# fanzhongyi/diffusion

Hardware: AMD Instinct MI355X
Metric: U-Net training images/sec @256 (SD-2-base U-Net, precomputed latents 4x32x32) (higher is better)
Workload: dtype bf16; 1 GPU; SD-2-base U-Net train step, latents 4x32x32, text 77x1024, batch 256/GPU (global 256), microbatch 256, AdamW, dp1; global_batch=256, microbatch=256, parallelism=dp1, params=865910724

## Files before the change

### diffusion_amd/_lib.py

```python
from __future__ import annotations

import ctypes as C
import os

_HERE = os.path.dirname(os.path.abspath(__file__))
LIB_PATH = os.path.join(_HERE, os.environ.get('DA_LIB_ALT') or 'libdiffusion_amd.so')

_vp, _l, _i, _f, _fp, _ll = C.c_void_p, C.c_long, C.c_int, C.c_float, C.c_void_p, C.c_void_p

SIGNATURES = {
    'da_gemm_nt': [_vp, _l, _vp, _vp, _l, _fp, _vp, _l, _vp, _l, _i, _i, _i, _i, _i, _i, _i, _i, _i, _i, _i, _f, _fp, _l,
                   _vp],
    'da_set_option': [C.c_char_p, _i],
    'da_gemm_nt_variant_for': [_i, _i, _i, _i, _l],
    'da_gemm_nt_geglu': [_vp, _l, _vp, _vp, _l, _vp, _l, _fp, _i, _i, _i, _vp],
    'da_gemm_nt_geglu_bwd': [_vp, _l, _vp, _vp, _l, _vp, _l, _i, _i, _i, _vp],
    'da_gemm_tn_wgrad': [_vp, _l, _vp, _l, _fp, _fp, _fp, _i, _i, _i, _i, _i, _i, _i, _i, _i, _fp, _l, _vp],
    'da_gemm_tn_variant_for': [_i, _i, _i, _i, _i, _i, _i, _i, _i],
    'da_attn_fwd': [_vp, _l, _vp, _l, _vp, _l, _vp, _l, _fp, _i, _i, _i, _i, _f, _vp],
    'da_attn_fwd_causal': [_vp, _l, _vp, _l, _vp, _l, _vp, _l, _fp, _i, _i, _i, _f, _vp],
    'da_attn_bwd': [_vp, _l, _vp, _l, _vp, _l, _vp, _l, _vp, _l, _fp, _fp, _vp, _l, _vp, _l, _vp, _l, _i, _i, _i, _i,
                    _f, _vp],
    'da_norm_scratch_floats': [_i, _i, _i],
    'da_groupnorm_fwd': [_vp, _l, _vp, _l, _fp, _fp, _fp, _fp, _fp, _i, _i, _i, _i, _f, _i, _vp],
    'da_groupnorm_bwd': [_vp, _l, _vp, _l, _vp, _l, _vp, _l, _fp, _fp, _fp, _fp, _fp, _fp, _fp, _i, _i, _i, _i, _i,
                         _vp],
    'da_groupnorm_plan_for': [_i, _i, _i, _i, _l, _l, _i, C.POINTER(_i)],
    'da_layernorm_fwd': [_vp, _l, _vp, _l, _fp, _fp, _fp, _i, _i, _f, _vp],
    'da_layernorm_bwd': [_vp, _l, _vp, _l, _vp, _l, _vp, _l, _fp, _fp, _fp, _fp, _fp, _i, _i, _vp],
    'da_colsum_accum': [_vp, _l, _fp, _fp, _i, _i, _vp],
    'da_image_colsum': [_vp, _l, _vp, _l, _fp, _fp, _i, _i, _i, _vp],
    'da_geglu_fwd': [_vp, _l, _vp, _l, _i, _i, _vp],
# ... 60 lines not shown
```

### diffusion_amd/csrc/gemm_tn.hip

```cpp
#include "common.hpp"
#include "diffusion_amd.h"

namespace {

struct GemmTNParams {
  const bf16* dY;
  const bf16* X;
  float* dW;
  long lddy, ldx;
  int M, N, Kt, Cin;
  int Hin, Win, Hout, Wout, ksize, mode;
  FastDiv div_hw, div_w;
  int tiles_n, tiles_k, splits, m_per_split;
  float* slab;
  int overwrite;
};

constexpr int TN_BM = 32;
constexpr int TN_LD = 288;
constexpr int TN_TILE = TN_BM * TN_LD;
constexpr int TN_STAGE = 2 * TN_TILE;
constexpr int TN_SMEM = 2 * TN_STAGE;

__global__ __launch_bounds__(256, 2) void gemm_tn_kernel(GemmTNParams p) {
// ... 153 lines not shown
      for (int u = 0; u < 8; ++u) acc[u] += *reinterpret_cast<const f32x4*>(src + (long)(sp + u) * 128 * 128);
    }
    for (int u = 0; sp < p.splits; ++sp, ++u) acc[u & 7] += *reinterpret_cast<const f32x4*>(src + (long)sp * 128 * 128);
    f32x4* dst = reinterpret_cast<f32x4*>(p.dW + (long)n * p.Kt + kc);
    const f32x4 sum = ((acc[0] + acc[1]) + (acc[2] + acc[3])) + ((acc[4] + acc[5]) + (acc[6] + acc[7]));
    *dst = p.overwrite ? sum : *dst + sum;
  }
}

}

int da_gemm_tn_v2_dispatch(int variant, const void* dY, long lddy, const void* X, long ldx, float* dW, float* dbias,
                           int M, int N, int Cin, int Hin, int Win, int Hout, int Wout, int ksize, int mode, float* ws,
                           long ws_floats, hipStream_t stream);
int da_gemm_tn_v2_fast_period(int M, int N, int Hin, int Win, int Hout, int Wout, int mode);
int g_tn_variant = 0;
int g_grad_overwrite = 0;

static bool tn_takes_v2(int M, int N, int Kt) {
  const bool big = (N >= 160) && (Kt >= 256) && (M >= 1024 || (M >= 256 && (long)N * Kt >= (8L << 20)));
  return g_tn_variant == 2 || g_tn_variant == 3 || (g_tn_variant == 0 && big);
}

extern "C" int da_gemm_tn_variant_for(int M, int N, int Cin, int Hin, int Win, int Hout, int Wout, int ksize, int mode) {
  if (!tn_takes_v2(M, N, ksize * ksize * Cin)) return 1;
  return da_gemm_tn_v2_fast_period(M, N, Hin, Win, Hout, Wout, mode) ? 3 : 2;
}

extern "C" int da_gemm_tn_wgrad(const void* dY, long lddy, const void* X, long ldx, float* dW, float* dbias,
                                float* scratch, int M, int N, int Cin, int Hin, int Win, int Hout, int Wout, int ksize,
// ... 39 lines not shown
  p.slab = nullptr;
  p.overwrite = g_grad_overwrite;
  if (splits > 1 && split_ws && (long)tiles * splits * 128 * 128 <= split_ws_floats && (p.Kt & 3) == 0) p.slab = split_ws;
  if (p.overwrite && splits > 1 && !p.slab)
    if (hipMemsetAsync(dW, 0, (size_t)N * p.Kt * sizeof(float), stream) != hipSuccess) return DA_ERR_LAUNCH;
  hipLaunchKernelGGL(gemm_tn_kernel, dim3(tiles * splits), dim3(256), 0, stream, p);
  DA_CHECK_LAUNCH();
  if (p.slab) {
    long blocks = ((long)p.N * (p.Kt >> 2) + 255) / 256;
    if (blocks > 2048) blocks = 2048;
    hipLaunchKernelGGL(tn1_slab_reduce_kernel, dim3((int)blocks), dim3(256), 0, stream, p);
    DA_CHECK_LAUNCH();
  }
  return DA_OK;
}
```

### diffusion_amd/csrc/gemm_tn_v2.hip

```cpp
#include "common.hpp"
#include "diffusion_amd.h"

int da_usable_cus(int cus);
extern int g_grad_overwrite;
int g_tn_ring = 0;


namespace {

struct GemmTN2Params {
  const bf16* dY;
  const bf16* X;
  float* dW;
  float* dbias;
  long lddy, ldx;
  int M, N, Kt, Cin;
  int Hin, Win, Hout, Wout, ksize, mode;
  FastDiv div_hw, div_w, div_cin;
  int tiles_n, tiles_k, splits, m_per_split;
  float* slab;
  float* bslab;
  int overwrite;
  int period;
  int ups64;
// ... 4 lines not shown
constexpr int T2_MS = 64;
constexpr int T2_BN = 320;
constexpr int T2_SA = T2_BN * 2;
constexpr int T2_A_BYTES = T2_MS * T2_SA;
constexpr int T2_AJ = T2_A_BYTES / 1024 / 8;

DEVINL int swA(int row) { return 2 * ((row >> 1) & 3); }
template <int BK>
DEVINL int swB(int row) { return (BK * 2) % 256 == 0 ? 2 * (row & 7) : 2 * ((row >> 1) & 3); }

DEVINL void glds16_tn(const void* gsrc, char* lds_dst) {
  __builtin_amdgcn_global_load_lds((const __attribute__((address_space(1))) void*)gsrc,
                                   (__attribute__((address_space(3))) void*)lds_dst, 16, 0, 0);
}

template <int T2_BK, bool FAST, bool CT, int RING = 0>
__global__ __launch_bounds__(512, 2) void gemm_tn2_kernel(GemmTN2Params p) {
  constexpr int T2_SB = T2_BK * 2;
  constexpr int T2_B_BYTES = T2_MS * T2_SB;
  constexpr int T2_STAGE = T2_A_BYTES + T2_B_BYTES;
  constexpr int T2_BJ = T2_B_BYTES / 1024 / 8;
  constexpr int C16B = T2_SB / 16;
  constexpr int JT = T2_BK / 32;
  extern __shared__ __attribute__((aligned(16))) char smem[];
  const int tid = threadIdx.x;
  const int lane = tid & 63;
  const int wave = __builtin_amdgcn_readfirstlane(tid >> 6);
  const int wa = wave >> 1, wb = wave & 1;

  int bid = blockIdx.x;
  {
    const int nblk = p.tiles_n * p.tiles_k * p.splits;
    const int q = nblk >> 3, r = nblk & 7;
    const int xcd = bid & 7, idx = bid >> 3;
    bid = (xcd < r ? xcd * (q + 1) : r * (q + 1) + (xcd - r) * q) + idx;
  }
  const int tk = bid % p.tiles_k;
  bid /= p.tiles_k;
  const int split = bid % p.splits;
  const int tn = bid / p.splits;
  const int n0 = tn * T2_BN, k0 = tk * T2_BK;
  const int m_begin = split * p.m_per_split;
  const int m_end = min(p.M, m_begin + p.m_per_split);
  const int nsteps = (m_end - m_begin + T2_MS - 1) / T2_MS;
  if (nsteps <= 0) return;
  const int HWo = p.Hout * p.Wout;
  const int pad = (p.ksize == 3) ? 1 : 0;
  const int gmul = (p.mode == 1) ? 2 : 1, gshift = (p.mode == 3) ? 1 : 0;
  const int hlim = (p.mode == 3) ? p.Hout : p.Hin, wlim = (p.mode == 3) ? p.Wout : p.Win;
  const char* zero = reinterpret_cast<const char*>(g_zero_page_tn);

  int mcur_f = m_begin;
  unsigned fa_off[T2_AJ], fx_off[T2_BJ], fx_off1[T2_BJ], fx_m0[T2_BJ], fx_m1[T2_BJ];
  const int src_step = (int)((long)T2_MS * p.Hin * p.Win / HWo);
  const long x_margin = (long)pad * (p.Win + 1);
// ... 221 lines not shown
#pragma unroll
      for (int i = 0; i < 5; ++i)
#pragma unroll
        for (int jj = 0; jj < JT / 2; ++jj)
          acc[i][jh * (JT / 2) + jj] =
              CT ? __builtin_amdgcn_mfma_f32_16x16x32_bf16(bfr[jj], a[i], acc[i][jh * (JT / 2) + jj], 0, 0, 0)
                 : __builtin_amdgcn_mfma_f32_16x16x32_bf16(a[i], bfr[jj], acc[i][jh * (JT / 2) + jj], 0, 0, 0);
    }
  };

  auto compute_half = [&](int stage, int ms) {
    const unsigned Ab = smem_off + stage * T2_STAGE;
    compute_half_at(Ab, Ab + T2_A_BYTES, ms);
  };

  if constexpr (RING > 0) {
    static_assert(!RING || (FAST && T2_BK == 192), "ring form: linear layers on the FAST path, 4 pieces per wave and half");
    constexpr int HALF_A = 32 * T2_SA, HALF = HALF_A + 32 * T2_SB;
    const int nh = (m_end - m_begin) >> 5;
    const bool is_a = wave < 5;
    unsigned off[4];
#pragma unroll
    for (int j = 0; j < 4; ++j) {
      if (is_a) {
        const int ci = (wave * 4 + j) * 64 + lane;
        const int row = ci / 40, pc = ci - row * 40;
        const int n = min(n0 + (pc ^ swA(row)) * 8, p.N - 8);
        off[j] = (unsigned)(row * (int)p.lddy + n);
      } else {
        const int ci = ((wave - 5) * 4 + j) * 64 + lane;
// ... 16 lines not shown
    };
#pragma unroll
    for (int h = 0; h < RING - 1; ++h) issue_half();
    int slot = 0;
    for (int h = 0; h < nh; ++h) {
      asm volatile("s_waitcnt vmcnt(%0)\n\ts_barrier" ::"n"(4 * (RING - 2)) : "memory");
      issue_half();
      const unsigned Ab = smem_off + slot * HALF;
      compute_half_at(Ab, Ab + HALF_A, 0);
      slot = slot + 1 == RING ? 0 : slot + 1;
    }
    asm volatile("s_waitcnt vmcnt(0)" ::: "memory");
  } else if constexpr (FAST) {
    issue_fast(0, true);
    __syncthreads();
    for (int t = 0; t < nsteps; ++t) {
      issue_fast((t + 1) & 1, t + 1 < nsteps);
      compute_half(t & 1, 0);
      compute_half(t & 1, 1);
      __syncthreads();
    }
  } else {
    issue(0);
    __syncthreads();
    for (int t = 0; t < nsteps; ++t) {
      compute_half(t & 1, 0);
      if (t + 1 < nsteps) issue((t + 1) & 1);
      compute_half(t & 1, 1);
      __syncthreads();
    }
  }

  if constexpr (CT) {
#pragma unroll
    for (int i = 0; i < 5; ++i)
#pragma unroll
      for (int j = 0; j < JT; ++j) {
        const int nl = wa * 80 + i * 16 + (lane & 15), kl = wb * (16 * JT) + j * 16 + (lane >> 4) * 4;
        const int n = n0 + nl, kc = k0 + kl;
        if (p.slab && p.splits > 1) {
          *reinterpret_cast<f32x4*>(p.slab + (((long)(tn * p.tiles_k + tk) * p.splits + split) * T2_BN + nl) * T2_BK + kl) = acc[i][j];
        } else if (n < p.N && kc < p.Kt) {
          float* dst = p.dW + (long)n * p.Kt + kc;
          if (p.splits == 1) {
            if (p.overwrite) *reinterpret_cast<f32x4*>(dst) = acc[i][j];
            else *reinterpret_cast<f32x4*>(dst) += acc[i][j];
          } else {
#pragma unroll
            for (int e = 0; e < 4; ++e) unsafeAtomicAdd(dst + e, acc[i][j][e]);
          }
        }
      }
    if (do_bias && lane < 16) {
#pragma unroll
      for (int i = 0; i < 5; ++i) {
        const int nl = wa * 80 + i * 16 + lane, n = n0 + nl;
        if (p.slab && p.splits > 1) p.bslab[((long)tn * p.splits + split) * T2_BN + nl] = accb[i][0];
        else if (n < p.N) {
          if (p.splits == 1) p.dbias[n] = p.overwrite ? accb[i][0] : p.dbias[n] + accb[i][0];
          else unsafeAtomicAdd(p.dbias + n, accb[i][0]);
        }
      }
    }
    return;
  }
#pragma unroll
  for (int i = 0; i < 5; ++i)
#pragma unroll
    for (int j = 0; j < JT; ++j) {
      const int kc = k0 + wb * (16 * JT) + j * 16 + (lane & 15);
#pragma unroll
      for (int e = 0; e < 4; ++e) {
        const int n = n0 + wa * 80 + i * 16 + (lane >> 4) * 4 + e;
        if (p.slab && p.splits > 1) {
          const int nl = wa * 80 + i * 16 + (lane >> 4) * 4 + e, kl = wb * (16 * JT) + j * 16 + (lane & 15);
          p.slab[(((long)(tn * p.tiles_k + tk) * p.splits + split) * T2_BN + nl) * T2_BK + kl] = acc[i][j][e];
        } else if (n < p.N && kc < p.Kt) {
          float* dst = p.dW + (long)n * p.Kt + kc;
          if (p.splits == 1) *dst = p.overwrite ? acc[i][j][e] : *dst + acc[i][j][e];
          else unsafeAtomicAdd(dst, acc[i][j][e]);
        }
      }
    }
  if (do_bias && (lane & 15) == 0) {
#pragma unroll
    for (int i = 0; i < 5; ++i)
#pragma unroll
      for (int e = 0; e < 4; ++e) {
        const int nl = wa * 80 + i * 16 + (lane >> 4) * 4 + e, n = n0 + nl;
        if (p.slab && p.splits > 1) p.bslab[((long)tn * p.splits + split) * T2_BN + nl] = accb[i][e];
        else if (n < p.N) {
          if (p.splits == 1) p.dbias[n] = p.overwrite ? accb[i][e] : p.dbias[n] + accb[i][e];
          else unsafeAtomicAdd(p.dbias + n, accb[i][e]);
        }
      }
  }
}

template <int BK>
__global__ __launch_bounds__(256) void tn_slab_reduce_kernel(GemmTN2Params p, int main_blocks) {
  if ((int)blockIdx.x >= main_blocks) {
    const int grp = threadIdx.x >> 4, l = threadIdx.x & 15;
    const int n = ((int)blockIdx.x - main_blocks) * 16 + grp;
    if (n < p.N) {
      const int tn = n / T2_BN;
      const float* src = p.bslab + ((long)tn * p.splits) * T2_BN + (n - tn * T2_BN);
      float a0 = 0.f, a1 = 0.f;
      int sp = l;
      for (; sp + 16 < p.splits; sp += 32) {
        a0 += src[(long)sp * T2_BN];
// ... 17 lines not shown
    f32x4 acc[8];
#pragma unroll
    for (int u = 0; u < 8; ++u) acc[u] = f32x4{0.f, 0.f, 0.f, 0.f};
    int sp = 0;
    for (; sp + 7 < p.splits; sp += 8) {
#pragma unroll
      for (int u = 0; u < 8; ++u) acc[u] += *reinterpret_cast<const f32x4*>(src + (long)(sp + u) * T2_BN * BK);
    }
    for (int u = 0; sp < p.splits; ++sp, ++u) acc[u & 7] += *reinterpret_cast<const f32x4*>(src + (long)sp * T2_BN * BK);
    f32x4* dst = reinterpret_cast<f32x4*>(p.dW + (long)n * p.Kt + kc);
    const f32x4 sum = ((acc[0] + acc[1]) + (acc[2] + acc[3])) + ((acc[4] + acc[5]) + (acc[6] + acc[7]));
    *dst = p.overwrite ? sum : *dst + sum;
  }
}

template <int BK, bool FAST>
int launch_tn2(GemmTN2Params p, float* ws, long ws_floats, hipStream_t stream) {
  constexpr int SMEM = 2 * (T2_A_BYTES + T2_MS * BK * 2);
  p.tiles_n = (p.N + T2_BN - 1) / T2_BN;
  p.tiles_k = (p.Kt + BK - 1) / BK;
  const int tiles = p.tiles_n * p.tiles_k;
  const int ncu = da_usable_cus(256);
  int best = 1;
  if (tiles < (ncu * 29) / 32) {
    int kcap = p.M / 6000;
    const int one_round = (ncu + tiles - 1) / tiles;
    if (kcap < one_round) kcap = one_round;
    const int max_splits = p.M / 512 > 0 ? p.M / 512 : 1;
    if (kcap > max_splits) kcap = max_splits;
    double best_eff = -1.0;
    bool found = false;
    for (int k = 1; k <= kcap; ++k) {
      const long blocks = (long)tiles * k;
      const double eff = (double)blocks / (double)(((blocks + ncu - 1) / ncu) * ncu);
      if (eff >= 0.9 && blocks >= ncu - 6) {
        best = k;
        found = true;
        break;
      }
      if (eff >= best_eff - 1e-9) {
        best_eff = eff;
        best = k;
      }
    }
    (void)found;
  }
  int mps = (p.M + best - 1) / best;
  mps = ((mps + T2_MS - 1) / T2_MS) * T2_MS;
  p.splits = (p.M + mps - 1) / mps;
  p.m_per_split = mps;
  static unsigned long long attr_done = 0, attr_done_ct = 0;
  if (da_ensure_dyn_smem((const void*)gemm_tn2_kernel<BK, FAST, false>, SMEM, &attr_done) != DA_OK) return DA_ERR_LAUNCH;
  if (da_ensure_dyn_smem((const void*)gemm_tn2_kernel<BK, FAST, true>, SMEM, &attr_done_ct) != DA_OK) return DA_ERR_LAUNCH;
  p.slab = p.bslab = nullptr;
  {
    const long tile_floats = (long)tiles * p.splits * T2_BN * BK;
    const long bias_floats = p.dbias ? (long)p.tiles_n * p.splits * T2_BN : 0;
    if (p.splits > 1 && ws && tile_floats + bias_floats <= ws_floats && (p.Kt & 3) == 0) {
      p.slab = ws;
      p.bslab = ws + tile_floats;
    }
// ... 59 lines not shown
  p.dY = (const bf16*)dY; p.X = (const bf16*)X; p.dW = dW; p.dbias = dbias;
  p.lddy = lddy; p.ldx = ldx;
  p.M = M; p.N = N; p.Cin = Cin; p.Kt = ksize * ksize * Cin;
  p.Hin = Hin; p.Win = Win; p.Hout = Hout; p.Wout = Wout; p.ksize = ksize; p.mode = mode;
  p.div_hw = make_fastdiv((unsigned)(Hout * Wout));
  p.div_w = make_fastdiv((unsigned)Wout);
  p.div_cin = make_fastdiv((unsigned)Cin);
  p.tiles_n = p.tiles_k = p.splits = p.m_per_split = 0;
  p.slab = p.bslab = nullptr;
  p.overwrite = 0;
  (void)variant;
  p.period = da_gemm_tn_v2_fast_period(M, N, Hin, Win, Hout, Wout, mode);
  p.ups64 = (p.period && mode == 3 && Wout == T2_MS) ? 1 : 0;
  return p.period ? launch_tn2<192, true>(p, ws, ws_floats, stream) : launch_tn2<192, false>(p, ws, ws_floats, stream);
}
```

### diffusion_amd/models/unet.py

```python
from __future__ import annotations

import math
import os
from dataclasses import dataclass
from typing import Dict, List, Optional, Tuple

import torch
import torch.nn as nn

from .. import ops
from ..ops import BF16, F32, Geom


@dataclass
class UNetConfig:
    in_channels: int = 4
    out_channels: int = 4
    block_out_channels: Tuple[int, ...] = (320, 640, 1280, 1280)
    attention_head_dim: Tuple[int, ...] = (5, 10, 20, 20)
    cross_attention_dim: int = 1024
    layers_per_block: int = 2
    norm_num_groups: int = 32
    norm_eps: float = 1e-5
    sample_size: int = 64
# ... 229 lines not shown
        fp = self.fp
        self.master = torch.zeros(fp.total, device=dev, dtype=F32)
        self.grad = torch.zeros(fp.total, device=dev, dtype=F32)
        self.exp_avg = torch.zeros(fp.total, device=dev, dtype=F32)
        self.exp_avg_sq = torch.zeros(fp.total, device=dev, dtype=F32)
        self.shadow = torch.zeros(fp.total, device=dev, dtype=BF16)
        self.shadow_t = torch.zeros(max(fp.total_t, 8), device=dev, dtype=BF16)
        self._bind_views()
        self._scratch = None
        self._scratch_key = None
        self.opt_step = 0
        self._grad_fresh = False
        self._grad_ready_cb = None
        import os
        self.wgrad_stream = torch.cuda.Stream() if os.environ.get('DA_WGRAD_STREAM', '0') == '1' else None
        self._tape = None
        if init:
            self.reset_parameters(seed)

    def _bind_views(self):
        fp = self.fp
        self._mats: Dict[str, Mat] = {}
        self._vecs: Dict[str, Vec] = {}
        for name, st in fp.storages.items():
            sl = slice(st.off, st.off + st.numel)
            if st.ntc is not None:
                N, T, C = st.ntc
                m = Mat()
                m.N, m.T, m.C = N, T, C
                m.w = self.shadow[sl].view(N, T * C)
# ... 147 lines not shown
            return
        main = torch.cuda.current_stream()
        ev = torch.cuda.Event()
        ev.record(main)
        ws.wait_event(ev)
        dy.record_stream(ws)
        x.record_stream(ws)
        with torch.cuda.stream(ws):
            old = ops.SPLITK_WS
            ops.SPLITK_WS = self._wgrad_ws
            try:
                ops.gemm_tn_wgrad(dy, x, gw, g, dbias=dbias, scratch=self._wgrad_scratch if scratch is not None else None)
            finally:
                ops.SPLITK_WS = old

    def _lin_fwd(self, x, key, out=None, bias=True, residual=None):
        m = self.M(key + '.weight')
        M = x.shape[0]
        y = out if out is not None else self._bf(M, m.N)
        ops.gemm_nt(x, m.w, y, Geom.linear(M), bias=self.V(key + '.bias').p if bias else None, residual=residual)
        return y

    def _lin_bwd(self, x, dy, key, bias=True, need_dx=True, dx_out=None):
        m = self.M(key + '.weight')
        M = x.shape[0]
        if _DGRAD_FIRST and need_dx:
            dx = dx_out if dx_out is not None else self._bf(M, m.C)
            ops.gemm_nt(dy, m.wt, dx, Geom.linear(M))
            self._wgrad(dy, x, m.gw, Geom.linear(M), dbias=self.V(key + '.bias').g if bias else None, scratch=self._scratch)
            return dx
        self._wgrad(dy, x, m.gw, Geom.linear(M), dbias=self.V(key + '.bias').g if bias else None,
                          scratch=self._scratch)
        if not need_dx:
            return None
        dx = dx_out if dx_out is not None else self._bf(M, m.C)
        ops.gemm_nt(dy, m.wt, dx, Geom.linear(M))
        return dx

    def _resnet_fwd(self, p, x, B, H, W, out=None):
        cfg = self.cfg
# ... 92 lines not shown
            ops.geglu_fwd(f, gg)
        h3 = self._lin_fwd(gg, tb + '.ff.net.2', residual=h2)
        y = self._lin_fwd(h3, p + '.proj_out', out=out, residual=x)
        saved = (p, x, gst, g, h0, ln1, n1, qkv, o1, l1, h1, ln2, n2, q2, kv2, o2, l2, h2, ln3, n3, f, gg, h3, B, H, W,
                 heads)
        return y, saved

    def _transformer_bwd(self, saved, dout):
        (p, x, gst, g, h0, ln1, n1, qkv, o1, l1, h1, ln2, n2, q2, kv2, o2, l2, h2, ln3, n3, f, gg, h3, B, H, W,
         heads) = saved
        HW = H * W
        M = B * HW
        C = x.shape[1]
        tb = p + '.transformer_blocks.0'
        nk = self._ctx.shape[0] // B
        dh3 = self._lin_bwd(h3, dout, p + '.proj_out')
        df = self._bf(M, 8 * C)
        if ops.geglu_bwd_fusable(4 * C, C):
            self._lin_bwd(gg, dh3, tb + '.ff.net.2', need_dx=False)
            ops.gemm_nt_geglu_bwd(dh3, self.M(tb + '.ff.net.2.weight').wt, f, df)
        else:
            dgg = self._lin_bwd(gg, dh3, tb + '.ff.net.2')
            ops.geglu_bwd(f, dgg, df)
            del dgg
        dn3 = self._lin_bwd(n3, df, tb + '.ff.net.0.proj')
        del df
        dh2 = self._ln_bwd(h2, dn3, dh3, tb + '.norm3', ln3)
        do2 = self._lin_bwd(o2, dh2, tb + '.attn2.to_out.0')
        dq2 = self._bf(M, C)
        dkv2 = self._bf(B * nk, 2 * C)
        ops.attn_bwd(q2, kv2[:, :C], kv2[:, C:], o2, do2, l2, self._delta, dq2, dkv2[:, :C], dkv2[:, C:], B, heads, HW,
                     nk, 0.125)
        self._wgrad(dkv2, self._ctx, self.M(tb + '.attn2.kv.weight').gw, Geom.linear(B * nk))
        dn2 = self._lin_bwd(n2, dq2, tb + '.attn2.to_q', bias=False)
        dh1 = self._ln_bwd(h1, dn2, dh2, tb + '.norm2', ln2)
        do1 = self._lin_bwd(o1, dh1, tb + '.attn1.to_out.0')
        dqkv = self._bf(M, 3 * C)
        ops.attn_bwd(qkv[:, :C], qkv[:, C:2 * C], qkv[:, 2 * C:], o1, do1, l1, self._delta, dqkv[:, :C],
                     dqkv[:, C:2 * C], dqkv[:, 2 * C:], B, heads, HW, HW, 0.125)
        mq = self.M(tb + '.attn1.qkv.weight')
        self._wgrad(dqkv, n1, mq.gw, Geom.linear(M))
        dn1 = self._bf(M, C)
        ops.gemm_nt(dqkv, mq.wt, dn1, Geom.linear(M))
        dh0 = self._ln_bwd(h0, dn1, dh1, tb + '.norm1', ln1)
        dg = self._lin_bwd(g, dh0, p + '.proj_in')
        return self._gn_bwd(x, dg, dout, p + '.norm', gst, B, HW, 0)

    def forward_features(self, xt8: torch.Tensor, t: torch.Tensor, ctx: torch.Tensor, B: int, S: int):
        cfg = self.cfg
        boc = cfg.block_out_channels
        n = len(boc)
        self._ensure_scratch(B, S)
        self._ctx = ctx
        tape: List[Tuple[str, tuple]] = []
        te0 = self._bf(B, boc[0])
        if t.dtype == F32:
            ops.timestep_embed_f32(t, te0)
        else:
            ops.timestep_embed(t, te0)
        te1 = self._lin_fwd(te0, 'time_embedding.linear_1')
# ... 216 lines not shown
```

### diffusion_amd/ops.py

```python
from __future__ import annotations

import ctypes
import os
from typing import Optional, Tuple

import torch

from . import _lib

BF16 = torch.bfloat16
F32 = torch.float32


def _stream() -> int:
    return torch.cuda.current_stream().cuda_stream


SPLITK_WS = None


PROFILE = None


class _Timed:
# ... 181 lines not shown
    if M != g.B * g.Hout * g.Wout or X.shape[0] != g.B * g.Hin * g.Win:
        raise ValueError('wgrad: row counts do not match the geometry')
    if dW.dtype != F32 or not dW.is_contiguous() or dW.numel() != N * g.ksize * g.ksize * Cin:
        raise ValueError(f'dW must be contiguous fp32 with {N * g.ksize * g.ksize * Cin} elements')
    mode = g.mode
    if mode == 2:
        raise ValueError('wgrad has no mode 2')
    with _Timed('gemm_tn', 2.0 * M * N * g.ksize * g.ksize * Cin, (M, N, g.ksize * g.ksize * Cin, g.ksize, g.mode)):
        db = _vec(dbias, N, 'dbias') if dbias is not None else 0
        sc = _f32buf(scratch, 256 * N * 2, 'scratch') if dbias is not None else 0
        _lib.call('da_gemm_tn_wgrad', dy_ptr, lddy, x_ptr, ldx, dW.data_ptr(), db, sc, M, N, Cin, g.Hin, g.Win,
                  g.Hout, g.Wout, g.ksize, mode, SPLITK_WS.data_ptr() if SPLITK_WS is not None else 0,
                  SPLITK_WS.numel() if SPLITK_WS is not None else 0, _stream())


def attn_fwd(Q, K, V, O, L2, B, H, Nq, Nk, scale):
    q, ldq = _mat(Q, BF16, 'Q')
    k, ldk = _mat(K, BF16, 'K')
    v, ldv = _mat(V, BF16, 'V')
    o, ldo = _mat(O, BF16, 'O')
    for t, n in ((Q, Nq), (O, Nq), (K, Nk), (V, Nk)):
        if tuple(t.shape) != (B * n, H * 64):
            raise ValueError(f'attention operand shape {tuple(t.shape)} != {(B * n, H * 64)}')
    with _Timed('attn_fwd', 4.0 * B * H * Nq * Nk * 64, (B, H, Nq, Nk, 0)):
        _lib.call('da_attn_fwd', q, ldq, k, ldk, v, ldv, o, ldo, _f32buf(L2, B * H * Nq, 'L2'), B, H, Nq, Nk,
                  float(scale), _stream())


def attn_fwd_causal(Q, K, V, O, L2, B, H, N, scale):
    q, ldq = _mat(Q, BF16, 'Q')
# ... 283 lines not shown
```

### include/diffusion_amd.h

```cpp
#ifndef DIFFUSION_AMD_H
#define DIFFUSION_AMD_H

#ifdef __cplusplus
extern "C" {
#endif

typedef struct ihipStream_t* da_stream_t;

int da_gemm_nt(const void* A, long lda, const void* W, void* C, long ldc, const float* bias, const void* rowbias,
               long ldrb, const void* R, long ldr, int M, int N, int K, int Cin, int Hin, int Win, int Hout, int Wout,
               int ksize, int mode, int out_fp32, float alpha, float* splitk_ws, long splitk_ws_floats,
               da_stream_t stream);

int da_gemm_nt_geglu(const void* A, long lda, const void* W, void* F, long ldf, void* G, long ldg, const float* bias,
                     int M, int inner, int K, da_stream_t stream);

int da_gemm_nt_geglu_bwd(const void* dY, long lddy, const void* Wt, const void* F, long ldf, void* dF, long lddf, int M,
                         int inner, int K, da_stream_t stream);

int da_set_option(const char* key, int value);
int da_gemm_nt_variant_for(int M, int N, int K, int Cin, long splitk_ws_floats);

int da_gemm_tn_wgrad(const void* dY, long lddy, const void* X, long ldx, float* dW, float* dbias, float* scratch, int M,
                     int N, int Cin, int Hin, int Win, int Hout, int Wout, int ksize, int mode, float* split_ws,
                     long split_ws_floats, da_stream_t stream);

int da_gemm_tn_variant_for(int M, int N, int Cin, int Hin, int Win, int Hout, int Wout, int ksize, int mode);

int da_attn_fwd(const void* Q, long ldq, const void* K, long ldk, const void* V, long ldv, void* O, long ldo,
                float* L2, int B, int H, int Nq, int Nk, float scale, da_stream_t stream);
int da_attn_fwd_causal(const void* Q, long ldq, const void* K, long ldk, const void* V, long ldv, void* O, long ldo,
                       float* L2, int B, int H, int N, float scale, da_stream_t stream);
int da_attn_bwd(const void* Q, long ldq, const void* K, long ldk, const void* V, long ldv, const void* O, long ldo,
                const void* dO, long lddo, const float* L2, float* Delta, void* dQ, long lddq, void* dK, long lddk,
                void* dV, long lddv, int B, int H, int Nq, int Nk, float scale, da_stream_t stream);

long da_norm_scratch_floats(int B, int HW, int C);

int da_groupnorm_fwd(const void* X, long ldx, void* Y, long ldy, const float* gamma, const float* beta,
                     float* mean_rstd, float* scale_shift, float* scratch, int B, int HW, int C, int G, float eps,
// ... 64 lines not shown
```

Baseline: 1538 images/sec.

## Batch transformer-block weight-gradient GEMMs into one grouped split-K launch

Defers the weight-gradient GEMMs of each transformer block's linear layers (proj_in/out, attention projections, FF) and runs them together in one grouped TN kernel, followed by a single split-K reduction kernel. Tiles from all problems share one grid, so the GPU fills better than with many small separate launches, and per-launch overhead drops. The tile kernel also gains a periodic accumulator flush into the slab or output during the main loop. The costs are extra workspace traffic, keeping activations alive longer, and more complex dispatch with a fallback to per-problem launches.

```diff
diff --git a/diffusion_amd/_lib.py b/diffusion_amd/_lib.py
--- a/diffusion_amd/_lib.py
+++ b/diffusion_amd/_lib.py
@@ -16,6 +16,7 @@
     'da_gemm_nt_geglu': [_vp, _l, _vp, _vp, _l, _vp, _l, _fp, _i, _i, _i, _vp],
     'da_gemm_nt_geglu_bwd': [_vp, _l, _vp, _vp, _l, _vp, _l, _i, _i, _i, _vp],
     'da_gemm_tn_wgrad': [_vp, _l, _vp, _l, _fp, _fp, _fp, _i, _i, _i, _i, _i, _i, _i, _i, _i, _fp, _l, _vp],
+    'da_gemm_tn_wgrad_grouped': [_vp, _i, _i, _fp, _l, _vp],
     'da_gemm_tn_variant_for': [_i, _i, _i, _i, _i, _i, _i, _i, _i],
     'da_attn_fwd': [_vp, _l, _vp, _l, _vp, _l, _vp, _l, _fp, _i, _i, _i, _i, _f, _vp],
     'da_attn_fwd_causal': [_vp, _l, _vp, _l, _vp, _l, _vp, _l, _fp, _i, _i, _i, _f, _vp],
diff --git a/diffusion_amd/csrc/gemm_tn.hip b/diffusion_amd/csrc/gemm_tn.hip
--- a/diffusion_amd/csrc/gemm_tn.hip
+++ b/diffusion_amd/csrc/gemm_tn.hip
@@ -191,6 +191,7 @@
                            int M, int N, int Cin, int Hin, int Win, int Hout, int Wout, int ksize, int mode, float* ws,
                            long ws_floats, hipStream_t stream);
 int da_gemm_tn_v2_fast_period(int M, int N, int Hin, int Win, int Hout, int Wout, int mode);
+int da_gemm_tn_v2_group(const DaWgradProblem* pr, int n, int M, float* ws, long ws_floats, hipStream_t stream);
 int g_tn_variant = 0;
 int g_grad_overwrite = 0;
 
@@ -260,3 +261,37 @@
   }
   return DA_OK;
 }
+
+extern "C" int da_gemm_tn_wgrad_grouped(const DaWgradProblem* pr, int n, int M, float* ws, long ws_floats, hipStream_t stream) {
+  DA_CLEAR_ERR();
+  if (!pr || n <= 0 || M <= 0 || M >= (1 << 24)) return DA_ERR_SHAPE;
+  if (!ws) ws_floats = 0;
+  bool group = g_tn_variant == 0;
+  for (int i = 0; i < n; ++i) {
+    const DaWgradProblem& q = pr[i];
+    if (!q.dY || !q.X || !q.dW || q.N <= 0 || q.Cin <= 0) return DA_ERR_SHAPE;
+    if ((q.N & 7) || (q.Cin & 7) || (q.lddy & 7) || (q.ldx & 7)) return DA_ERR_SHAPE;
+    group = group && tn_takes_v2(M, q.N, q.Cin) && da_gemm_tn_v2_fast_period(M, q.N, 1, 1, 1, 1, 0) != 0;
+  }
+  if (group) {
+    const int rc = da_gemm_tn_v2_group(pr, n, M, ws, ws_floats, stream);
+    if (rc >= 0) return rc;
+  }
+  for (int i = 0; i < n; ++i) {
+    const DaWgradProblem& q = pr[i];
+    float* scratch = nullptr;
+    float* sws = ws;
+    long sws_floats = ws_floats;
+    if (q.dbias && !tn_takes_v2(M, q.N, q.Cin)) {
+      const long need = 256L * q.N * 2;
+      if (ws_floats < need) return DA_ERR_SHAPE;
+      scratch = ws;
+      sws = ws + need;
+      sws_floats = ws_floats - need;
+    }
+    const int rc = da_gemm_tn_wgrad(q.dY, q.lddy, q.X, q.ldx, q.dW, q.dbias, scratch, M, q.N, q.Cin, 1, 1, 1, 1, 1, 0,
+                                    sws_floats > 0 ? sws : nullptr, sws_floats, stream);
+    if (rc) return rc;
+  }
+  return DA_OK;
+}
diff --git a/diffusion_amd/csrc/gemm_tn_v2.hip b/diffusion_amd/csrc/gemm_tn_v2.hip
--- a/diffusion_amd/csrc/gemm_tn_v2.hip
+++ b/diffusion_amd/csrc/gemm_tn_v2.hip
@@ -1,3 +1,5 @@
+#include <string.h>
+
 #include "common.hpp"
 #include "diffusion_amd.h"
 
@@ -42,8 +44,9 @@
                                    (__attribute__((address_space(3))) void*)lds_dst, 16, 0, 0);
 }
 
-template <int T2_BK, bool FAST, bool CT, int RING = 0>
-__global__ __launch_bounds__(512, 2) void gemm_tn2_kernel(GemmTN2Params p) {
+template <int T2_BK, bool FAST, bool CT, int RING = 0, int FLUSH = 0>
+DEVINL void gemm_tn2_tile(const GemmTN2Params& p, const int tn, const int tk, const int split, float* const slab_tile,
+                          float* const bslab_tile) {
   constexpr int T2_SB = T2_BK * 2;
   constexpr int T2_B_BYTES = T2_MS * T2_SB;
   constexpr int T2_STAGE = T2_A_BYTES + T2_B_BYTES;
@@ -56,17 +59,6 @@
   const int wave = __builtin_amdgcn_readfirstlane(tid >> 6);
   const int wa = wave >> 1, wb = wave & 1;
 
-  int bid = blockIdx.x;
-  {
-    const int nblk = p.tiles_n * p.tiles_k * p.splits;
-    const int q = nblk >> 3, r = nblk & 7;
-    const int xcd = bid & 7, idx = bid >> 3;
-    bid = (xcd < r ? xcd * (q + 1) : r * (q + 1) + (xcd - r) * q) + idx;
-  }
-  const int tk = bid % p.tiles_k;
-  bid /= p.tiles_k;
-  const int split = bid % p.splits;
-  const int tn = bid / p.splits;
   const int n0 = tn * T2_BN, k0 = tk * T2_BK;
   const int m_begin = split * p.m_per_split;
   const int m_end = min(p.M, m_begin + p.m_per_split);
@@ -318,6 +310,43 @@
     compute_half_at(Ab, Ab + T2_A_BYTES, ms);
   };
 
+  auto ct_store = [&](const bool first) {
+    int ln = lane;
+    if constexpr (FLUSH > 0) asm volatile("" : "+v"(ln));
+#pragma unroll
+    for (int i = 0; i < 5; ++i)
+#pragma unroll
+      for (int j = 0; j < JT; ++j) {
+        const int nl = wa * 80 + i * 16 + (ln & 15), kl = wb * (16 * JT) + j * 16 + (ln >> 4) * 4;
+        const int n = n0 + nl, kc = k0 + kl;
+        if (slab_tile) {
+          f32x4* sdst = reinterpret_cast<f32x4*>(slab_tile + (long)nl * T2_BK + kl);
+          if (first) *sdst = acc[i][j];
+          else *sdst += acc[i][j];
+        } else if (n < p.N && kc < p.Kt) {
+          float* dst = p.dW + (long)n * p.Kt + kc;
+          if (p.splits == 1) {
+            if (p.overwrite && first) *reinterpret_cast<f32x4*>(dst) = acc[i][j];
+            else *reinterpret_cast<f32x4*>(dst) += acc[i][j];
+          } else {
+#pragma unroll
+            for (int e = 0; e < 4; ++e) unsafeAtomicAdd(dst + e, acc[i][j][e]);
+          }
+        }
+      }
+    if (do_bias && ln < 16) {
+#pragma unroll
+      for (int i = 0; i < 5; ++i) {
+        const int nl = wa * 80 + i * 16 + ln, n = n0 + nl;
+        if (slab_tile) bslab_tile[nl] = first ? accb[i][0] : bslab_tile[nl] + accb[i][0];
+        else if (n < p.N) {
+          if (p.splits == 1) p.dbias[n] = (p.overwrite && first) ? accb[i][0] : p.dbias[n] + accb[i][0];
+          else unsafeAtomicAdd(p.dbias + n, accb[i][0]);
+        }
+      }
+    }
+  };
+  bool first_store = true;
   if constexpr (RING > 0) {
     static_assert(!RING || (FAST && T2_BK == 192), "ring form: linear layers on the FAST path, 4 pieces per wave and half");
     constexpr int HALF_A = 32 * T2_SA, HALF = HALF_A + 32 * T2_SB;
@@ -364,11 +393,26 @@
   } else if constexpr (FAST) {
     issue_fast(0, true);
     __syncthreads();
+    [[maybe_unused]] int since_flush = 0;
     for (int t = 0; t < nsteps; ++t) {
       issue_fast((t + 1) & 1, t + 1 < nsteps);
       compute_half(t & 1, 0);
       compute_half(t & 1, 1);
       __syncthreads();
+      if constexpr (FLUSH > 0) {
+        static_assert(FLUSH == 0 || (CT && RING == 0), "the flush goes through the transposed-product epilogue");
+        if (++since_flush == FLUSH || t + 1 == nsteps) {
+          ct_store(first_store);
+          first_store = false;
+          since_flush = 0;
+#pragma unroll
+          for (int i = 0; i < 5; ++i) {
+            accb[i] = f32x4{0.f, 0.f, 0.f, 0.f};
+#pragma unroll
+            for (int j = 0; j < JT; ++j) acc[i][j] = f32x4{0.f, 0.f, 0.f, 0.f};
+          }
+        }
+      }
     }
   } else {
     issue(0);
@@ -382,36 +426,7 @@
   }
 
   if constexpr (CT) {
-#pragma unroll
-    for (int i = 0; i < 5; ++i)
-#pragma unroll
-      for (int j = 0; j < JT; ++j) {
-        const int nl = wa * 80 + i * 16 + (lane & 15), kl = wb * (16 * JT) + j * 16 + (lane >> 4) * 4;
-        const int n = n0 + nl, kc = k0 + kl;
-        if (p.slab && p.splits > 1) {
-          *reinterpret_cast<f32x4*>(p.slab + (((long)(tn * p.tiles_k + tk) * p.splits + split) * T2_BN + nl) * T2_BK + kl) = acc[i][j];
-        } else if (n < p.N && kc < p.Kt) {
-          float* dst = p.dW + (long)n * p.Kt + kc;
-          if (p.splits == 1) {
-            if (p.overwrite) *reinterpret_cast<f32x4*>(dst) = acc[i][j];
-            else *reinterpret_cast<f32x4*>(dst) += acc[i][j];
-          } else {
-#pragma unroll
-            for (int e = 0; e < 4; ++e) unsafeAtomicAdd(dst + e, acc[i][j][e]);
-          }
-        }
-      }
-    if (do_bias && lane < 16) {
-#pragma unroll
-      for (int i = 0; i < 5; ++i) {
-        const int nl = wa * 80 + i * 16 + lane, n = n0 + nl;
-        if (p.slab && p.splits > 1) p.bslab[((long)tn * p.splits + split) * T2_BN + nl] = accb[i][0];
-        else if (n < p.N) {
-          if (p.splits == 1) p.dbias[n] = p.overwrite ? accb[i][0] : p.dbias[n] + accb[i][0];
-          else unsafeAtomicAdd(p.dbias + n, accb[i][0]);
-        }
-      }
-    }
+    if constexpr (FLUSH == 0) ct_store(first_store);
     return;
   }
 #pragma unroll
@@ -422,9 +437,9 @@
 #pragma unroll
       for (int e = 0; e < 4; ++e) {
         const int n = n0 + wa * 80 + i * 16 + (lane >> 4) * 4 + e;
-        if (p.slab && p.splits > 1) {
+        if (slab_tile) {
           const int nl = wa * 80 + i * 16 + (lane >> 4) * 4 + e, kl = wb * (16 * JT) + j * 16 + (lane & 15);
-          p.slab[(((long)(tn * p.tiles_k + tk) * p.splits + split) * T2_BN + nl) * T2_BK + kl] = acc[i][j][e];
+          slab_tile[(long)nl * T2_BK + kl] = acc[i][j][e];
         } else if (n < p.N && kc < p.Kt) {
           float* dst = p.dW + (long)n * p.Kt + kc;
           if (p.splits == 1) *dst = p.overwrite ? acc[i][j][e] : *dst + acc[i][j][e];
@@ -438,12 +453,135 @@
 #pragma unroll
       for (int e = 0; e < 4; ++e) {
         const int nl = wa * 80 + i * 16 + (lane >> 4) * 4 + e, n = n0 + nl;
-        if (p.slab && p.splits > 1) p.bslab[((long)tn * p.splits + split) * T2_BN + nl] = accb[i][e];
+        if (slab_tile) bslab_tile[nl] = accb[i][e];
         else if (n < p.N) {
           if (p.splits == 1) p.dbias[n] = p.overwrite ? accb[i][e] : p.dbias[n] + accb[i][e];
           else unsafeAtomicAdd(p.dbias + n, accb[i][e]);
         }
       }
+  }
+}
+
+DEVINL int xcd_run_id(int bid, int nblk) {
+  const int q = nblk >> 3, r = nblk & 7;
+  const int xcd = bid & 7, idx = bid >> 3;
+  return (xcd < r ? xcd * (q + 1) : r * (q + 1) + (xcd - r) * q) + idx;
+}
+
+template <int T2_BK, bool FAST, bool CT, int RING = 0>
+__global__ __launch_bounds__(512, 2) void gemm_tn2_kernel(GemmTN2Params p) {
+  int bid = xcd_run_id(blockIdx.x, p.tiles_n * p.tiles_k * p.splits);
+  const int tk = bid % p.tiles_k;
+  bid /= p.tiles_k;
+  const int split = bid % p.splits;
+  const int tn = bid / p.splits;
+  float* slab_tile = nullptr;
+  float* bslab_tile = nullptr;
+  if (p.slab && p.splits > 1) {
+    slab_tile = p.slab + ((long)(tn * p.tiles_k + tk) * p.splits + split) * T2_BN * T2_BK;
+    bslab_tile = p.bslab + ((long)tn * p.splits + split) * T2_BN;
+  }
+  gemm_tn2_tile<T2_BK, FAST, CT, RING>(p, tn, tk, split, slab_tile, bslab_tile);
+}
+
+constexpr int TG_MAX_PROBLEMS = 12;
+constexpr int TG_MAX_SEGS = TG_MAX_PROBLEMS + 1;
+constexpr int TG_BK = 192;
+constexpr int TG_FLUSH = 48;
+constexpr int TG_RED_BLOCKS = T2_BN * TG_BK / 4 / 256;
+
+struct TnGroupSeg {
+  const bf16* dY;
+  const bf16* X;
+  float* dW;
+  float* dbias;
+  float* slab;
+  float* bslab;
+  long lddy, ldx;
+  FastDiv div_cin;
+  int N, Cin, tiles_k;
+  int tile0, ntiles;
+  int splits, m_per_split;
+  int wg0;
+  int red0;
+};
+
+struct TnGroupParams {
+  TnGroupSeg seg[TG_MAX_SEGS];
+  int nseg, M, overwrite;
+  int wg_unsplit, wg_total;
+};
+
+__global__ __launch_bounds__(512, 2) void gemm_tn2_group_kernel(TnGroupParams g) {
+  int bid = blockIdx.x;
+  bid = bid < g.wg_unsplit ? xcd_run_id(bid, g.wg_unsplit) : g.wg_unsplit + xcd_run_id(bid - g.wg_unsplit, g.wg_total - g.wg_unsplit);
+  TnGroupSeg sg = g.seg[0];
+#pragma unroll
+  for (int i = 1; i < TG_MAX_SEGS; ++i)
+    if (i < g.nseg && bid >= g.seg[i].wg0) sg = g.seg[i];
+  const int lid = bid - sg.wg0;
+  const int split = lid / sg.ntiles;
+  const int trel = lid - split * sg.ntiles;
+  const int tn = (sg.tile0 + trel) / sg.tiles_k, tk = (sg.tile0 + trel) - tn * sg.tiles_k;
+  GemmTN2Params p;
+  p.dY = sg.dY; p.X = sg.X; p.dW = sg.dW; p.dbias = sg.dbias;
+  p.lddy = sg.lddy; p.ldx = sg.ldx;
+  p.M = g.M; p.N = sg.N; p.Kt = sg.Cin; p.Cin = sg.Cin;
+  p.Hin = p.Win = p.Hout = p.Wout = 1; p.ksize = 1; p.mode = 0;
+  p.div_hw.magic = p.div_w.magic = (1ull << 40) + 1ull;
+  p.div_hw.d = p.div_w.d = 1u;
+  p.div_cin = sg.div_cin;
+  p.tiles_n = 0; p.tiles_k = sg.tiles_k; p.splits = sg.splits; p.m_per_split = sg.m_per_split;
+  p.slab = sg.slab; p.bslab = sg.bslab;
+  p.overwrite = g.overwrite;
+  p.period = 1; p.ups64 = 0;
+  const long part = (long)trel * sg.splits + split;
+  gemm_tn2_tile<TG_BK, true, true, 0, TG_FLUSH>(p, tn, tk, split, sg.splits > 1 ? sg.slab + part * (T2_BN * TG_BK) : nullptr,
+                                               sg.splits > 1 ? sg.bslab + part * T2_BN : nullptr);
+}
+
+__global__ __launch_bounds__(256) void tn_group_reduce_kernel(TnGroupParams g) {
+  const int bid = blockIdx.x;
+  TnGroupSeg sg = g.seg[0];
+#pragma unroll
+  for (int i = 1; i < TG_MAX_SEGS; ++i)
+    if (i < g.nseg && bid >= g.seg[i].red0) sg = g.seg[i];
+  const int lb = bid - sg.red0;
+  const int trel = lb / TG_RED_BLOCKS, chunk = lb - trel * TG_RED_BLOCKS;
+  const int tn = (sg.tile0 + trel) / sg.tiles_k, tk = (sg.tile0 + trel) - tn * sg.tiles_k;
+  const int e = chunk * 256 + threadIdx.x;
+  const int nl = e / (TG_BK / 4), kl = (e - nl * (TG_BK / 4)) * 4;
+  const int n = tn * T2_BN + nl, kc = tk * TG_BK + kl;
+  if (n < sg.N && kc < sg.Cin) {
+    const float* src = sg.slab + (((long)trel * sg.splits) * T2_BN + nl) * TG_BK + kl;
+    f32x4 acc[8];
+#pragma unroll
+    for (int u = 0; u < 8; ++u) acc[u] = f32x4{0.f, 0.f, 0.f, 0.f};
+    int sp = 0;
+    for (; sp + 7 < sg.splits; sp += 8) {
+#pragma unroll
+      for (int u = 0; u < 8; ++u) acc[u] += *reinterpret_cast<const f32x4*>(src + (long)(sp + u) * T2_BN * TG_BK);
+    }
+    for (int u = 0; sp < sg.splits; ++sp, ++u) acc[u & 7] += *reinterpret_cast<const f32x4*>(src + (long)sp * T2_BN * TG_BK);
+    f32x4* dst = reinterpret_cast<f32x4*>(sg.dW + (long)n * sg.Cin + kc);
+    const f32x4 sum = ((acc[0] + acc[1]) + (acc[2] + acc[3])) + ((acc[4] + acc[5]) + (acc[6] + acc[7]));
+    *dst = g.overwrite ? sum : *dst + sum;
+  }
+  if (chunk == 0 && tk == 0 && sg.dbias) {
+    for (int bl = threadIdx.x; bl < T2_BN; bl += 256) {
+      const int bn = tn * T2_BN + bl;
+      if (bn >= sg.N) break;
+      const float* src = sg.bslab + ((long)trel * sg.splits) * T2_BN + bl;
+      float a0 = 0.f, a1 = 0.f;
+      int sp = 0;
+      for (; sp + 1 < sg.splits; sp += 2) {
+        a0 += src[(long)sp * T2_BN];
+        a1 += src[(long)(sp + 1) * T2_BN];
+      }
+      if (sp < sg.splits) a0 += src[(long)sp * T2_BN];
+      const float a = a0 + a1;
+      sg.dbias[bn] = g.overwrite ? a : sg.dbias[bn] + a;
+    }
   }
 }
 
@@ -491,37 +629,38 @@
   }
 }
 
+int tn2_pick_splits(int tiles, int M, int ncu) {
+  int best = 1;
+  if (tiles < (ncu * 29) / 32) {
+    int kcap = M / 6000;
+    const int one_round = (ncu + tiles - 1) / tiles;
+    if (kcap < one_round) kcap = one_round;
+    const int max_splits = M / 512 > 0 ? M / 512 : 1;
+    if (kcap > max_splits) kcap = max_splits;
+    double best_eff = -1.0;
+    for (int k = 1; k <= kcap; ++k) {
+      const long blocks = (long)tiles * k;
+      const double eff = (double)blocks / (double)(((blocks + ncu - 1) / ncu) * ncu);
+      if (eff >= 0.9 && blocks >= ncu - 6) {
+        best = k;
+        break;
+      }
+      if (eff >= best_eff - 1e-9) {
+        best_eff = eff;
+        best = k;
+      }
+    }
+  }
+  return best;
+}
+
 template <int BK, bool FAST>
 int launch_tn2(GemmTN2Params p, float* ws, long ws_floats, hipStream_t stream) {
   constexpr int SMEM = 2 * (T2_A_BYTES + T2_MS * BK * 2);
   p.tiles_n = (p.N + T2_BN - 1) / T2_BN;
   p.tiles_k = (p.Kt + BK - 1) / BK;
   const int tiles = p.tiles_n * p.tiles_k;
-  const int ncu = da_usable_cus(256);
-  int best = 1;
-  if (tiles < (ncu * 29) / 32) {
-    int kcap = p.M / 6000;
-    const int one_round = (ncu + tiles - 1) / tiles;
-    if (kcap < one_round) kcap = one_round;
-    const int max_splits = p.M / 512 > 0 ? p.M / 512 : 1;
-    if (kcap > max_splits) kcap = max_splits;
-    double best_eff = -1.0;
-    bool found = false;
-    for (int k = 1; k <= kcap; ++k) {
-      const long blocks = (long)tiles * k;
-      const double eff = (double)blocks / (double)(((blocks + ncu - 1) / ncu) * ncu);
-      if (eff >= 0.9 && blocks >= ncu - 6) {
-        best = k;
-        found = true;
-        break;
-      }
-      if (eff >= best_eff - 1e-9) {
-        best_eff = eff;
-        best = k;
-      }
-    }
-    (void)found;
-  }
+  const int best = tn2_pick_splits(tiles, p.M, da_usable_cus(256));
   int mps = (p.M + best - 1) / best;
   mps = ((mps + T2_MS - 1) / T2_MS) * T2_MS;
   p.splits = (p.M + mps - 1) / mps;
@@ -611,3 +750,77 @@
   p.ups64 = (p.period && mode == 3 && Wout == T2_MS) ? 1 : 0;
   return p.period ? launch_tn2<192, true>(p, ws, ws_floats, stream) : launch_tn2<192, false>(p, ws, ws_floats, stream);
 }
+
+int da_gemm_tn_v2_group(const DaWgradProblem* pr, int n, int M, float* ws, long ws_floats, hipStream_t stream) {
+  if (n < 2 || n > TG_MAX_PROBLEMS || g_tn_ring) return -1;
+  const int ncu = da_usable_cus(256);
+  int tiles_k[TG_MAX_PROBLEMS], tiles[TG_MAX_PROBLEMS], first[TG_MAX_PROBLEMS];
+  int total = 0;
+  for (int i = 0; i < n; ++i) {
+    first[i] = total;
+    if (pr[i].lddy >= (1L << 24) || pr[i].ldx >= (1L << 24)) return -1;
+    tiles_k[i] = (pr[i].Cin + TG_BK - 1) / TG_BK;
+    tiles[i] = ((pr[i].N + T2_BN - 1) / T2_BN) * tiles_k[i];
+    total += tiles[i];
+  }
+  const int rest = total % ncu;
+  const int k = rest ? tn2_pick_splits(rest, M, ncu) : 1;
+  int mps = (M + k - 1) / k;
+  mps = ((mps + T2_MS - 1) / T2_MS) * T2_MS;
+  const int splits = (M + mps - 1) / mps;
+  const int unsplit = splits > 1 ? total - rest : total;
+  const long slab_floats = (long)(total - unsplit) * splits * T2_BN * TG_BK;
+  const long bslab_floats = (long)(total - unsplit) * splits * T2_BN;
+  if (splits > 1 && (!ws || slab_floats + bslab_floats > ws_floats)) return -1;
+
+  TnGroupParams g;
+  memset(&g, 0, sizeof(g));
+  g.M = M;
+  g.overwrite = g_grad_overwrite;
+  g.wg_unsplit = unsplit;
+  int nseg = 0, t_done = 0, wg = unsplit, red = 0;
+  long part = 0;
+  for (int pass = 0; pass < 2; ++pass) {
+    int wg_u = 0;
+    for (int i = 0; i < n; ++i) {
+      int border = unsplit - first[i];
+      border = border < 0 ? 0 : (border > tiles[i] ? tiles[i] : border);
+      const int lo = pass == 0 ? 0 : border, hi = pass == 0 ? border : tiles[i];
+      if (hi <= lo) continue;
+      TnGroupSeg& s = g.seg[nseg++];
+      s.dY = (const bf16*)pr[i].dY; s.X = (const bf16*)pr[i].X; s.dW = pr[i].dW; s.dbias = pr[i].dbias;
+      s.lddy = pr[i].lddy; s.ldx = pr[i].ldx;
+      s.div_cin = make_fastdiv((unsigned)pr[i].Cin);
+      s.N = pr[i].N; s.Cin = pr[i].Cin; s.tiles_k = tiles_k[i];
+      s.tile0 = lo; s.ntiles = hi - lo;
+      if (pass == 0) {
+        s.splits = 1; s.m_per_split = M;
+        s.slab = s.bslab = nullptr;
+        s.wg0 = wg_u; s.red0 = 0;
+        wg_u += s.ntiles;
+      } else {
+        s.splits = splits; s.m_per_split = mps;
+        s.slab = ws + part * (T2_BN * TG_BK);
+        s.bslab = ws + slab_floats + part * T2_BN;
+        s.wg0 = wg; s.red0 = red;
+        wg += s.ntiles * splits;
+        red += s.ntiles * TG_RED_BLOCKS;
+        part += (long)s.ntiles * splits;
+      }
+      t_done += s.ntiles;
+    }
+  }
+  if (t_done != total || nseg > TG_MAX_SEGS) return DA_ERR_LAUNCH;
+  g.nseg = nseg;
+  g.wg_total = wg;
+  constexpr int SMEM = 2 * (T2_A_BYTES + T2_MS * TG_BK * 2);
+  static unsigned long long attr_done = 0;
+  if (da_ensure_dyn_smem((const void*)gemm_tn2_group_kernel, SMEM, &attr_done) != DA_OK) return DA_ERR_LAUNCH;
+  hipLaunchKernelGGL(gemm_tn2_group_kernel, dim3(g.wg_total), dim3(512), SMEM, stream, g);
+  DA_CHECK_LAUNCH();
+  if (red > 0) {
+    hipLaunchKernelGGL(tn_group_reduce_kernel, dim3(red), dim3(256), 0, stream, g);
+    DA_CHECK_LAUNCH();
+  }
+  return DA_OK;
+}
diff --git a/diffusion_amd/models/unet.py b/diffusion_amd/models/unet.py
--- a/diffusion_amd/models/unet.py
+++ b/diffusion_amd/models/unet.py
@@ -267,6 +267,7 @@
         self._grad_ready_cb = None
         import os
         self.wgrad_stream = torch.cuda.Stream() if os.environ.get('DA_WGRAD_STREAM', '0') == '1' else None
+        self.wgrad_group = os.environ.get('DA_WGRAD_GROUP', '1') != '0'
         self._tape = None
         if init:
             self.reset_parameters(seed)
@@ -444,6 +445,26 @@
             finally:
                 ops.SPLITK_WS = old
 
+    def _wgrad_grouped(self, jobs):
+        ws = self.wgrad_stream
+        if ws is None:
+            ops.gemm_tn_wgrad_grouped(jobs)
+            return
+        main = torch.cuda.current_stream()
+        ev = torch.cuda.Event()
+        ev.record(main)
+        ws.wait_event(ev)
+        for dy, x, _, _ in jobs:
+            dy.record_stream(ws)
+            x.record_stream(ws)
+        with torch.cuda.stream(ws):
+            old = ops.SPLITK_WS
+            ops.SPLITK_WS = self._wgrad_ws
+            try:
+                ops.gemm_tn_wgrad_grouped(jobs)
+            finally:
+                ops.SPLITK_WS = old
+
     def _lin_fwd(self, x, key, out=None, bias=True, residual=None):
         m = self.M(key + '.weight')
         M = x.shape[0]
@@ -451,9 +472,16 @@
         ops.gemm_nt(x, m.w, y, Geom.linear(M), bias=self.V(key + '.bias').p if bias else None, residual=residual)
         return y
 
-    def _lin_bwd(self, x, dy, key, bias=True, need_dx=True, dx_out=None):
+    def _lin_bwd(self, x, dy, key, bias=True, need_dx=True, dx_out=None, defer=None):
         m = self.M(key + '.weight')
         M = x.shape[0]
+        if defer is not None:
+            defer.append((dy, x, m.gw, self.V(key + '.bias').g if bias else None))
+            if not need_dx:
+                return None
+            dx = dx_out if dx_out is not None else self._bf(M, m.C)
+            ops.gemm_nt(dy, m.wt, dx, Geom.linear(M))
+            return dx
         if _DGRAD_FIRST and need_dx:
             dx = dx_out if dx_out is not None else self._bf(M, m.C)
             ops.gemm_nt(dy, m.wt, dx, Geom.linear(M))
@@ -576,36 +604,42 @@
         C = x.shape[1]
         tb = p + '.transformer_blocks.0'
         nk = self._ctx.shape[0] // B
-        dh3 = self._lin_bwd(h3, dout, p + '.proj_out')
+        jobs = [] if self.wgrad_group else None
+        dh3 = self._lin_bwd(h3, dout, p + '.proj_out', defer=jobs)
         df = self._bf(M, 8 * C)
         if ops.geglu_bwd_fusable(4 * C, C):
-            self._lin_bwd(gg, dh3, tb + '.ff.net.2', need_dx=False)
+            self._lin_bwd(gg, dh3, tb + '.ff.net.2', need_dx=False, defer=jobs)
             ops.gemm_nt_geglu_bwd(dh3, self.M(tb + '.ff.net.2.weight').wt, f, df)
         else:
-            dgg = self._lin_bwd(gg, dh3, tb + '.ff.net.2')
+            dgg = self._lin_bwd(gg, dh3, tb + '.ff.net.2', defer=jobs)
             ops.geglu_bwd(f, dgg, df)
             del dgg
-        dn3 = self._lin_bwd(n3, df, tb + '.ff.net.0.proj')
+        dn3 = self._lin_bwd(n3, df, tb + '.ff.net.0.proj', defer=jobs)
         del df
         dh2 = self._ln_bwd(h2, dn3, dh3, tb + '.norm3', ln3)
-        do2 = self._lin_bwd(o2, dh2, tb + '.attn2.to_out.0')
+        do2 = self._lin_bwd(o2, dh2, tb + '.attn2.to_out.0', defer=jobs)
         dq2 = self._bf(M, C)
         dkv2 = self._bf(B * nk, 2 * C)
         ops.attn_bwd(q2, kv2[:, :C], kv2[:, C:], o2, do2, l2, self._delta, dq2, dkv2[:, :C], dkv2[:, C:], B, heads, HW,
                      nk, 0.125)
         self._wgrad(dkv2, self._ctx, self.M(tb + '.attn2.kv.weight').gw, Geom.linear(B * nk))
-        dn2 = self._lin_bwd(n2, dq2, tb + '.attn2.to_q', bias=False)
+        dn2 = self._lin_bwd(n2, dq2, tb + '.attn2.to_q', bias=False, defer=jobs)
         dh1 = self._ln_bwd(h1, dn2, dh2, tb + '.norm2', ln2)
-        do1 = self._lin_bwd(o1, dh1, tb + '.attn1.to_out.0')
+        do1 = self._lin_bwd(o1, dh1, tb + '.attn1.to_out.0', defer=jobs)
         dqkv = self._bf(M, 3 * C)
         ops.attn_bwd(qkv[:, :C], qkv[:, C:2 * C], qkv[:, 2 * C:], o1, do1, l1, self._delta, dqkv[:, :C],
                      dqkv[:, C:2 * C], dqkv[:, 2 * C:], B, heads, HW, HW, 0.125)
         mq = self.M(tb + '.attn1.qkv.weight')
-        self._wgrad(dqkv, n1, mq.gw, Geom.linear(M))
+        if jobs is not None:
+            jobs.append((dqkv, n1, mq.gw, None))
+        else:
+            self._wgrad(dqkv, n1, mq.gw, Geom.linear(M))
         dn1 = self._bf(M, C)
         ops.gemm_nt(dqkv, mq.wt, dn1, Geom.linear(M))
         dh0 = self._ln_bwd(h0, dn1, dh1, tb + '.norm1', ln1)
-        dg = self._lin_bwd(g, dh0, p + '.proj_in')
+        dg = self._lin_bwd(g, dh0, p + '.proj_in', defer=jobs)
+        if jobs:
+            self._wgrad_grouped(jobs)
         return self._gn_bwd(x, dg, dout, p + '.norm', gst, B, HW, 0)
 
     def forward_features(self, xt8: torch.Tensor, t: torch.Tensor, ctx: torch.Tensor, B: int, S: int):
diff --git a/diffusion_amd/ops.py b/diffusion_amd/ops.py
--- a/diffusion_amd/ops.py
+++ b/diffusion_amd/ops.py
@@ -219,6 +219,33 @@
                   SPLITK_WS.numel() if SPLITK_WS is not None else 0, _stream())
 
 
+class _WgradProblem(ctypes.Structure):
+    _fields_ = [('dY', ctypes.c_void_p), ('lddy', ctypes.c_long), ('X', ctypes.c_void_p), ('ldx', ctypes.c_long),
+                ('dW', ctypes.c_void_p), ('dbias', ctypes.c_void_p), ('N', ctypes.c_int), ('Cin', ctypes.c_int)]
+
+
+def gemm_tn_wgrad_grouped(jobs):
+    if not jobs:
+        return
+    M = jobs[0][0].shape[0]
+    arr = (_WgradProblem * len(jobs))()
+    flops = 0.0
+    for q, (dY, X, dW, dbias) in zip(arr, jobs):
+        q.dY, q.lddy = _mat(dY, BF16, 'dY')
+        q.X, q.ldx = _mat(X, BF16, 'X')
+        N, Cin = dY.shape[1], X.shape[1]
+        if dY.shape[0] != M or X.shape[0] != M:
+            raise ValueError('grouped wgrad: every dY and X must have the same number of rows')
+        if dW.dtype != F32 or not dW.is_contiguous() or dW.numel() != N * Cin or not dW.is_cuda:
+            raise ValueError(f'dW must be contiguous fp32 with {N * Cin} elements')
+        q.dW, q.dbias, q.N, q.Cin = dW.data_ptr(), (_vec(dbias, N, 'dbias') or None), N, Cin
+        flops += 2.0 * M * N * Cin
+    with _Timed('gemm_tn', flops, (M, len(jobs), int(flops / (2.0 * M)), 1, 'group')):
+        _lib.call('da_gemm_tn_wgrad_grouped', ctypes.cast(arr, ctypes.c_void_p), len(jobs), M,
+                  SPLITK_WS.data_ptr() if SPLITK_WS is not None else 0,
+                  SPLITK_WS.numel() if SPLITK_WS is not None else 0, _stream())
+
+
 def attn_fwd(Q, K, V, O, L2, B, H, Nq, Nk, scale):
     q, ldq = _mat(Q, BF16, 'Q')
     k, ldk = _mat(K, BF16, 'K')
diff --git a/include/diffusion_amd.h b/include/diffusion_amd.h
--- a/include/diffusion_amd.h
+++ b/include/diffusion_amd.h
@@ -24,6 +24,18 @@
 int da_gemm_tn_wgrad(const void* dY, long lddy, const void* X, long ldx, float* dW, float* dbias, float* scratch, int M,
                      int N, int Cin, int Hin, int Win, int Hout, int Wout, int ksize, int mode, float* split_ws,
                      long split_ws_floats, da_stream_t stream);
+
+typedef struct DaWgradProblem {
+  const void* dY;
+  long lddy;
+  const void* X;
+  long ldx;
+  float* dW;
+  float* dbias;
+  int N, Cin;
+} DaWgradProblem;
+
+int da_gemm_tn_wgrad_grouped(const DaWgradProblem* problems, int n, int M, float* ws, long ws_floats, da_stream_t stream);
 
 int da_gemm_tn_variant_for(int M, int N, int Cin, int Hin, int Win, int Hout, int Wout, int ksize, int mode);
 
```

New measurement: 1512 images/sec. -1.7%, worse.
